# fhfonsecaa/SG-GAN-TF2

Hardware: AMD Instinct MI355X
Metric: train-step images/sec (G+D fwd/bwd) at 512x256 (higher is better)
Workload: dtype bf16; 1 GPU; BASELINE configs[2]: cycle-mode train step (north_star unit: G_A->B + G_B->A + D_A + D_B, LSGAN + cycle-L1 + gradient-sensitive losses; 12G+14D conv MACs), 9-block ResNet generators, 512x256, batch 8/GPU, bf16 storage / f32 accumulate; mode=cycle, global_batch=8, height=256, width=512, parallelism=dp1, mixed_gradient_chain=False

## Files before the change

sg-gan-tf2_amd/csrc/common.h:

```cpp
#pragma once
#include <hip/hip_runtime.h>
#include <hip/hip_ext.h>
#include <stdint.h>
#include <atomic>
#include <type_traits>
#include "../../include/sggan.h"

typedef __bf16 bf16;
typedef __attribute__((ext_vector_type(8))) __bf16 bf16x8;
typedef __attribute__((ext_vector_type(4))) __bf16 bf16x4;
typedef __attribute__((ext_vector_type(4))) float f32x4;
typedef __attribute__((ext_vector_type(4))) uint32_t u32x4;
typedef __attribute__((ext_vector_type(2))) uint32_t u32x2;

#define SGG_WAVE 64

template <typename T> struct ET;
template <> struct ET<float> {
    static constexpr int VEC = 4;
    __device__ static inline void unpack(const u32x4& c, float* f) {
#pragma unroll
        for (int i = 0; i < 4; ++i) f[i] = __uint_as_float(c[i]);
    }
    __device__ static inline u32x4 pack(const float* f) {
// ... 149 lines not shown
    const uint32_t m = __builtin_amdgcn_readfirstlane((uint32_t)(uintptr_t)lds_wave_base);
    const uint64_t b = (uint64_t)(uintptr_t)sbase;
    const uint64_t sb = (uint64_t)(uint32_t)__builtin_amdgcn_readfirstlane((uint32_t)b) |
                        ((uint64_t)(uint32_t)__builtin_amdgcn_readfirstlane((uint32_t)(b >> 32)) << 32);
    asm volatile("s_mov_b32 m0, %2\n\ts_nop 0\n\tglobal_load_lds_dwordx4 %0, %1" ::"v"(voff), "s"(sb), "s"(m) : "memory", "m0");
}

__device__ inline void dma4_to_lds(const void* gsrc, __attribute__((address_space(3))) void* lds_wave_base) {
    const uint32_t m = __builtin_amdgcn_readfirstlane((uint32_t)(uintptr_t)lds_wave_base);
    asm volatile("s_mov_b32 m0, %1\n\ts_nop 0\n\tglobal_load_lds_dword %0, off" ::"v"(gsrc), "s"(m) : "memory", "m0");
}
template <int N> __device__ inline void sgg_wait_vm() {
    static_assert(N >= 0 && N < 64, "vmcnt is a 6-bit counter");
    __builtin_amdgcn_s_waitcnt((N & 15) | ((N >> 4) << 14) | 0x0F70);
    asm volatile("" ::: "memory");
}
#define SGG_WAIT_VM0() sgg_wait_vm<0>()
#define SGG_WAIT_LGKM0() do { __builtin_amdgcn_s_waitcnt(0xC07F); asm volatile("" ::: "memory"); } while (0)

static inline int sgg_check_launch() { return hipGetLastError() == hipSuccess ? SGG_OK : SGG_ELAUNCH; }

static inline int sgg_lds_attr(const void* kern, int bytes, std::atomic<uint64_t>& done) {
    int dev = 0;
    if (hipGetDevice(&dev) != hipSuccess) return SGG_ELAUNCH;
    const uint64_t bit = 1ull << (dev & 63);
    if (done.load(std::memory_order_acquire) & bit) return SGG_OK;
    if (hipFuncSetAttribute(kern, hipFuncAttributeMaxDynamicSharedMemorySize, bytes) != hipSuccess) { (void)hipGetLastError(); return SGG_ELAUNCH; }
    done.fetch_or(bit, std::memory_order_release);
    return SGG_OK;
}
#define SGG_LDS_ATTR(kern, bytes)                                                        \
    do {                                                                                 \
        static std::atomic<uint64_t> sgg_attr_done_{0};                                  \
        int sgg_attr_rc_ = sgg_lds_attr((const void*)(kern), (int)(bytes), sgg_attr_done_); \
        if (sgg_attr_rc_) return sgg_attr_rc_;                                           \
    } while (0)

struct SggTimedLaunch { hipEvent_t start = nullptr, stop = nullptr; int consumed = 0; };
SggTimedLaunch& sgg_timed_launch();
template <typename F, typename... Args>
static inline void sgg_launch_timed(F kern, dim3 grid, dim3 block, unsigned lds, hipStream_t s, Args... args) {
    SggTimedLaunch& t = sgg_timed_launch();
    if (t.start && !t.consumed) {
        hipExtLaunchKernelGGL(kern, grid, block, lds, s, t.start, t.stop, 0, args...);
        t.consumed = 1;
    } else {
        hipLaunchKernelGGL(kern, grid, block, lds, s, args...);
    }
}

struct SggConfig {
    int halo3 = 1, s2halo = 1, w9 = 1, w9s2 = 1, stem_dgrad_halo = 1, wgrad_rowfast = 1, n7 = 1;
    int in_fused_maxhw = -1;
    int ablate = 0;
};
const SggConfig& sgg_config();
static inline size_t align_up(size_t v, size_t a) { return (v + a - 1) / a * a; }
```

sg-gan-tf2_amd/csrc/conv.hip:

```cpp
#include "conv_internal.h"

const SggConfig& sgg_config() {
#ifdef SGG_LAB
    static const SggConfig cfg = [] {
        SggConfig c;
        auto rd = [](const char* n, int dflt) { const char* e = getenv(n); return e ? atoi(e) : dflt; };
        c.halo3 = rd("SGG_HALO3", c.halo3);
        c.s2halo = rd("SGG_S2HALO", c.s2halo);
        c.w9 = rd("SGG_W9", c.w9);
        c.w9s2 = rd("SGG_W9S2", c.w9s2);
        c.stem_dgrad_halo = rd("SGG_STEM_DGRAD_HALO", c.stem_dgrad_halo);
        c.n7 = rd("SGG_N7", c.n7);
        c.wgrad_rowfast = rd("SGG_WGRAD_ROWFAST", c.wgrad_rowfast);
        c.in_fused_maxhw = rd("SGG_IN_FUSED_MAXHW", c.in_fused_maxhw);
        c.ablate = rd("SGG_ABLATE", 0);
        return c;
    }();
    return cfg;
#else
    static const SggConfig cfg;
    return cfg;
#endif
}

template <typename T>
__device__ inline u32x4 chunk_add(const u32x4& a, const u32x4& b) {
    float fa[ET<T>::VEC], fb[ET<T>::VEC];
    ET<T>::unpack(a, fa);
    ET<T>::unpack(b, fb);
#pragma unroll
    for (int i = 0; i < ET<T>::VEC; ++i) fa[i] += fb[i];
    return ET<T>::pack(fa);
}

__device__ inline int reflect_preimages(int h, int H, int p, int* j) {
    int n = 0;
    j[n++] = h + p;
    if (h >= 1 && h <= p) j[n++] = p - h;
    if (h >= H - 1 - p && h <= H - 2) j[n++] = p + 2 * (H - 1) - h;
    return n;
}

template <typename T, int BN, int WGM>
__global__ __launch_bounds__(256) void conv_border_fold_kernel(ConvArgs a) {
    constexpr int VEC = ET<T>::VEC;
    constexpr int ES = (int)sizeof(T);
    constexpr int BM = 64;
    constexpr int WGN = 4 / WGM;
    constexpr int WM = BM / WGM, WN = BN / WGN;
    constexpr int MI = WM / 16, NI = WN / 16;
    constexpr int PA = BM / 32;
    constexpr int QA = (BN + 31) / 32;
    static_assert(WM % 16 == 0 && WN % 16 == 0, "tile shape");

    extern __shared__ __attribute__((aligned(16))) char smem[];
    char* sP = smem;
    char* sQ = smem + BM * 128;

    const int tid = threadIdx.x, lane = tid & 63, wave = __builtin_amdgcn_readfirstlane(tid >> 6);
    const int wm = wave / WGN, wn = wave % WGN;
    const int SC = a.K, DC = a.C;
    const int cpv = SC / VEC;
    const int wrow = a.R * a.S * SC;
    const int p = a.pad_t, p2 = 2 * p;
    const int Bimg = p2 * a.W + (a.H - p2) * p2;
    const int M = a.N * Bimg;
    const int m0 = blockIdx.x * BM, n0 = blockIdx.y * BN;
// ... 2092 lines not shown
```

sg-gan-tf2_amd/csrc/norm.hip:

```cpp
#include "common.h"
#include <type_traits>

#define IN_U (BWD ? 2 : 4)
template <typename T> using InAcc = typename std::conditional<std::is_same<T, float>::value, double, float>::type;

struct InSplit { const float* gamma2; const float* beta2; float* dgamma2; float* dbeta2; int nsplit; };
static inline InSplit in_nosplit() { InSplit s; s.gamma2 = nullptr; s.beta2 = nullptr; s.dgamma2 = nullptr; s.dbeta2 = nullptr; s.nsplit = 0x7fffffff; return s; }

#ifndef IN_NT
#define IN_NT 15
#endif
template <typename T, typename TG, bool NT = false>
__device__ inline void in_load_grad(const char* dy, size_t elem, float* gv) {
    if constexpr (std::is_same<T, TG>::value) {
        ET<T>::unpack(NT ? ld16_nt(dy + elem * sizeof(T)) : ld16(dy + elem * sizeof(T)), gv);
    } else {
        static_assert(std::is_same<TG, float>::value && ET<T>::VEC == 8, "mixed mode: f32 gradient of a bf16 tensor");
        ET<float>::unpack(ld16(dy + elem * 4), gv);
        ET<float>::unpack(ld16(dy + elem * 4 + 16), gv + 4);
    }
}

static inline int in_rows_per_chunk(int64_t HW) {
    int64_t r = (HW + 127) / 128;
// ... 182 lines not shown
            auto sweep = [&](auto res_c) {
                constexpr bool RES = decltype(res_c)::value;
                auto one = [&](const u32x4& xr, const u32x4& rr, const float* gv, size_t off) {
                    float xv[VEC], o[VEC];
                    ET<T>::unpack(xr, xv);
                    if (!BWD) {
#pragma unroll
                        for (int e = 0; e < VEC; ++e) o[e] = act_apply_c<ACT>(xv[e] * A[e] + B[e], leak);
                        if (RES) {
                            float rv[VEC];
                            ET<T>::unpack(rr, rv);
#pragma unroll
                            for (int e = 0; e < VEC; ++e) o[e] += rv[e];
                        }
                    } else {
#pragma unroll
                        for (int e = 0; e < VEC; ++e) {
                            float xh = (xv[e] - mu[e]) * rs[e];
                            float g = gv[e] * act_grad_c<ACT>(gm[e] * xh + bt[e], leak);
                            o[e] = A[e] * (g - m1[e] - xh * m2[e]);
                        }
                    }
                    st16(out + off, ET<T>::pack(o));
                };
                const size_t base = ((size_t)n * HW * C + (size_t)cv * VEC) * sizeof(T), pstep = (size_t)C * sizeof(T);
                int64_t p = p0 + prow;
                for (; p + (IN_U - 1) * rows < p1; p += IN_U * rows) {
                    u32x4 xr[IN_U], rr[IN_U];
                    float gv[IN_U][BWD ? VEC : 1];
#pragma unroll
                    for (int u = 0; u < IN_U; ++u) {
                        const size_t off = base + (size_t)(p + u * rows) * pstep;
                        xr[u] = (IN_NT & (BWD ? 2 : 1)) ? ld16_nt(x + off) : ld16(x + off);
                        if (RES) rr[u] = (IN_NT & 8) ? ld16_nt(residual + off) : ld16(residual + off);
                    }
                    if (BWD) {
#pragma unroll
                        for (int u = 0; u < IN_U; ++u) in_load_grad<T, TG>(dy, (base + (size_t)(p + u * rows) * pstep) / sizeof(T), gv[u]);
                    }
#pragma unroll
                    for (int u = 0; u < IN_U; ++u) one(xr[u], rr[u], gv[u], base + (size_t)(p + u * rows) * pstep);
                }
                for (; p < p1; p += rows) {
                    const size_t off = base + (size_t)p * pstep;
                    float gv[BWD ? VEC : 1];
                    const u32x4 xr = (IN_NT & (BWD ? 2 : 1)) ? ld16_nt(x + off) : ld16(x + off);
                    u32x4 rr = xr;
                    if (RES) rr = (IN_NT & 8) ? ld16_nt(residual + off) : ld16(residual + off);
                    if (BWD) in_load_grad<T, TG, (IN_NT & 4) != 0>(dy, off / sizeof(T), gv);
                    one(xr, rr, gv, off);
                }
            };
            if (!BWD && residual) sweep(std::true_type{}); else sweep(std::false_type{});
        });
    }
}


#define IN_CVB 4
#define IN_FUSED_MAXHW 512

template <typename T, bool BWD>
__global__ __launch_bounds__(256) void in_fused_small_kernel(const char* x, const char* dy, const char* residual, const float* gamma,
                                                             const float* beta, float* stats, float* tot, char* out,
                                                             int64_t HW, int C, float eps, int act, float leak, InSplit sp) {
    constexpr int VEC = ET<T>::VEC;
    constexpr int ROWS = 256 / IN_CVB;
    const int CV = C / VEC;
    const int n = blockIdx.y;
    if (n >= sp.nsplit) { gamma = sp.gamma2; beta = sp.beta2; }
    const int cvl = threadIdx.x % IN_CVB, prow = threadIdx.x / IN_CVB;
    const int cv = blockIdx.x * IN_CVB + cvl;
    const bool live = cv < CV;
    using AccT = InAcc<T>;
    __shared__ AccT red[256][2 * VEC + 1];
    __shared__ float sh_a[IN_CVB * VEC], sh_b[IN_CVB * VEC];

    float mu[VEC], rs[VEC], gm[VEC], bt[VEC];
    if (live) {
#pragma unroll
        for (int e = 0; e < VEC; ++e) {
            const int c = cv * VEC + e;
            gm[e] = gamma[c]; bt[e] = beta[c];
            if (BWD) { mu[e] = stats[((size_t)n * C + c) * 2]; rs[e] = stats[((size_t)n * C + c) * 2 + 1]; }
        }
    }
    AccT s1[VEC], s2[VEC];
#pragma unroll
    for (int e = 0; e < VEC; ++e) s1[e] = s2[e] = (AccT)0;
    if (live)
        for (int64_t p = prow; p < HW; p += ROWS) {
            const size_t off = (((size_t)n * HW + p) * C + (size_t)cv * VEC) * sizeof(T);
            float xv[VEC];
            ET<T>::unpack(ld16(x + off), xv);
            if (!BWD) {
#pragma unroll
                for (int e = 0; e < VEC; ++e) { s1[e] += (AccT)xv[e]; s2[e] += (AccT)xv[e] * (AccT)xv[e]; }
            } else {
                float gv[VEC];
                ET<T>::unpack(ld16(dy + off), gv);
#pragma unroll
                for (int e = 0; e < VEC; ++e) {
                    const float xh = (xv[e] - mu[e]) * rs[e];
                    const float g = gv[e] * (act == SGG_ACT_RELU ? (gm[e] * xh + bt[e] > 0.f ? 1.f : 0.f) : act == SGG_ACT_LRELU ? (gm[e] * xh + bt[e] > 0.f ? 1.f : leak) : 1.f);
                    s1[e] += (AccT)g; s2[e] += (AccT)g * (AccT)xh;
                }
// ... 154 lines not shown
                    const u32x4 dzr = ET<T>::pack(dz);
                    st16(dz_out + off, dzr);
                    ET<T>::unpack(dzr, dz);
#pragma unroll
                    for (int e = 0; e < VEC; ++e) {
                        const float xh = (xv[e] - mu[e]) * rs[e];
                        s1[e] += (AccT)dz[e]; s2[e] += (AccT)dz[e] * (AccT)xh;
                    }
                };
                const size_t base = ((size_t)n * HW * C + (size_t)cv * VEC) * sizeof(T), pstep = (size_t)C * sizeof(T);
                int64_t p = p0 + prow;
                for (; p + rows < p1; p += 2 * rows) {
                    u32x4 xr[2], gr[2], yr[2];
#pragma unroll
                    for (int u = 0; u < 2; ++u) {
                        const size_t off = base + (size_t)(p + u * rows) * pstep;
                        xr[u] = ld16(x + off); gr[u] = ld16_nt(dy + off); yr[u] = ld16_nt(y + off);
                    }
#pragma unroll
                    for (int u = 0; u < 2; ++u) one(xr[u], gr[u], yr[u], base + (size_t)(p + u * rows) * pstep);
                }
                for (; p < p1; p += rows) {
                    const size_t off = base + (size_t)p * pstep;
                    one(ld16(x + off), ld16_nt(dy + off), ld16_nt(y + off), off);
                }
            });
        }
#pragma unroll
        for (int e = 0; e < VEC; ++e) { red[threadIdx.x][e] = s1[e]; red[threadIdx.x][VEC + e] = s2[e]; }
        __syncthreads();
        for (int item = threadIdx.x; item < lanes * VEC; item += 256) {
            const int l = item / VEC, e = item % VEC;
            AccT a = (AccT)0, b = (AccT)0;
            for (int r = 0; r < rows; ++r) { a += red[r * lanes + l][e]; b += red[r * lanes + l][VEC + e]; }
            const int c = (cvb + l) * VEC + e;
            const size_t o = (((size_t)n * chunks + chunk) * C + c) * 2;
            partial[o] = (float)a; partial[o + 1] = (float)b;
        }
        __syncthreads();
    }
}

static bool in_use_fused(int64_t HW) {
    const int mx = sgg_config().in_fused_maxhw;
    return HW <= (mx >= 0 ? mx : IN_FUSED_MAXHW);
}

static int in_rows_per_block(int N, int64_t HW, int C, int vec) {
    int64_t r = HW * N / 2048;
    if (r < 64) r = 64;
    if (r > 4096) r = 4096;
    return (int)r;
}

extern "C" {

size_t sgg_instnorm_workspace(int N, int64_t HW, int C) {
    if (N <= 0 || HW <= 0 || C <= 0) return 0;
    return ((size_t)N * in_chunks(HW) * C * 2 + (size_t)N * C * 4) * sizeof(float);
}

static int instnorm_fwd_impl(const void* x, const float* gamma, const float* beta, const void* residual, void* y, float* stats,
                     int N, int64_t HW, int C, float eps, int act, float leak, int dtype, void* ws, size_t ws_bytes, void* stream, InSplit sp) {
    if (!x || !gamma || !beta || !y || !stats || N <= 0 || HW <= 0 || C <= 0 || C % SGG_CPAD) return SGG_EINVAL;
    if (act == SGG_ACT_TANH) return SGG_EUNSUPPORTED;
    if (!ws || ws_bytes < sgg_instnorm_workspace(N, HW, C)) return SGG_EWORKSPACE;
    hipStream_t s = (hipStream_t)stream;
    if (dtype != SGG_BF16 && dtype != SGG_F32) return SGG_EINVAL;
    if (in_use_fused(HW)) {
        const int vec = dtype == SGG_BF16 ? 8 : 4;
        dim3 gf((unsigned)((C / vec + IN_CVB - 1) / IN_CVB), N);
        if (dtype == SGG_BF16) hipLaunchKernelGGL((in_fused_small_kernel<bf16, false>), gf, dim3(256), 0, s, (const char*)x, nullptr, (const char*)residual, gamma, beta, stats, nullptr, (char*)y, HW, C, eps, act, leak, sp);
        else hipLaunchKernelGGL((in_fused_small_kernel<float, false>), gf, dim3(256), 0, s, (const char*)x, nullptr, (const char*)residual, gamma, beta, stats, nullptr, (char*)y, HW, C, eps, act, leak, sp);
        return sgg_check_launch();
    }
    int chunks = in_chunks(HW);
    float* partial = (float*)ws;
    int rpb = in_rows_per_block(N, HW, C, 0);
    dim3 gp(chunks, N), ga((unsigned)((HW + rpb - 1) / rpb), N);
    if (dtype == SGG_BF16) {
        hipLaunchKernelGGL((in_partial_kernel<bf16, false>), gp, dim3(256), 0, s, (const char*)x, nullptr, gamma, beta, nullptr, partial, HW, C, chunks, in_rows_per_chunk(HW), act, leak, sp);
        hipLaunchKernelGGL(in_finalize_fwd_kernel, dim3((C + FIN_CH - 1) / FIN_CH, N), dim3(1024), 0, s, partial, stats, HW, C, chunks, eps);
        sgg_launch_timed(in_apply_kernel<bf16, false>, ga, dim3(256), 0u, s, (const char*)x, (const char*)nullptr, (const char*)residual, gamma, beta, (const float*)stats, (const float*)nullptr, (char*)y, HW, C, rpb, act, leak, InParamGrad{}, sp);
    } else if (dtype == SGG_F32) {
        hipLaunchKernelGGL((in_partial_kernel<float, false>), gp, dim3(256), 0, s, (const char*)x, nullptr, gamma, beta, nullptr, partial, HW, C, chunks, in_rows_per_chunk(HW), act, leak, sp);
        hipLaunchKernelGGL(in_finalize_fwd_kernel, dim3((C + FIN_CH - 1) / FIN_CH, N), dim3(1024), 0, s, partial, stats, HW, C, chunks, eps);
        hipLaunchKernelGGL((in_apply_kernel<float, false>), ga, dim3(256), 0, s, (const char*)x, nullptr, (const char*)residual, gamma, beta, stats, nullptr, (char*)y, HW, C, rpb, act, leak, InParamGrad{}, sp);
    } else return SGG_EINVAL;
    return sgg_check_launch();
}

static int instnorm_fwd_partial_impl(const void* x, const float* gamma, const float* beta, const void* residual, void* y, float* stats,
                             const float* partial, int chunks, int N, int64_t HW, int C, float eps, int act, float leak, int dtype,
                             void* stream, InSplit sp) {
    if (!x || !gamma || !beta || !y || !stats || !partial || chunks <= 0 || N <= 0 || HW <= 0 || C <= 0 || C % SGG_CPAD) return SGG_EINVAL;
    if (act == SGG_ACT_TANH) return SGG_EUNSUPPORTED;
    if (dtype != SGG_BF16 && dtype != SGG_F32) return SGG_EINVAL;
    hipStream_t s = (hipStream_t)stream;
    int rpb = in_rows_per_block(N, HW, C, 0);
    dim3 ga((unsigned)((HW + rpb - 1) / rpb), N);
    hipLaunchKernelGGL(in_finalize_fwd_kernel, dim3((C + FIN_CH - 1) / FIN_CH, N), dim3(1024), 0, s, partial, stats, HW, C, chunks, eps);
    if (dtype == SGG_BF16) sgg_launch_timed(in_apply_kernel<bf16, false>, ga, dim3(256), 0u, s, (const char*)x, (const char*)nullptr, (const char*)residual, gamma, beta, (const float*)stats, (const float*)nullptr, (char*)y, HW, C, rpb, act, leak, InParamGrad{}, sp);
    else hipLaunchKernelGGL((in_apply_kernel<float, false>), ga, dim3(256), 0, s, (const char*)x, nullptr, (const char*)residual, gamma, beta, stats, nullptr, (char*)y, HW, C, rpb, act, leak, InParamGrad{}, sp);
    return sgg_check_launch();
}

static int instnorm_bwd_impl(const void* dy, const void* x, const float* gamma, const float* beta, const float* stats, void* dx,
                     float* dgamma, float* dbeta, int N, int64_t HW, int C, int C_real, int accumulate, int act, float leak,
                     int dtype, void* ws, size_t ws_bytes, void* stream, InSplit sp) {
    if (!dy || !x || !gamma || !beta || !stats || !dx || !dgamma || !dbeta || N <= 0 || HW <= 0 || C <= 0 || C % SGG_CPAD || C_real <= 0 || C_real > C) return SGG_EINVAL;
    if (act == SGG_ACT_TANH) return SGG_EUNSUPPORTED;
    if (!ws || ws_bytes < sgg_instnorm_workspace(N, HW, C)) return SGG_EWORKSPACE;
    hipStream_t s = (hipStream_t)stream;
    int chunks = in_chunks(HW);
    float* partial = (float*)ws;
    float* sums = partial + (size_t)N * chunks * C * 2;
    float* tot = sums + (size_t)N * C * 2;
    int rpb = in_rows_per_block(N, HW, C, 0);
    dim3 gp(chunks, N), ga((unsigned)((HW + rpb - 1) / rpb), N);
    const InParamGrad pg{tot, dgamma, dbeta, N, C_real, accumulate};
    if (dtype != SGG_BF16 && dtype != SGG_F32) return SGG_EINVAL;
    if (in_use_fused(HW)) {
        const int vec = dtype == SGG_BF16 ? 8 : 4;
        dim3 gf((unsigned)((C / vec + IN_CVB - 1) / IN_CVB), N);
        if (dtype == SGG_BF16) hipLaunchKernelGGL((in_fused_small_kernel<bf16, true>), gf, dim3(256), 0, s, (const char*)x, (const char*)dy, nullptr, gamma, beta, (float*)stats, tot, (char*)dx, HW, C, 0.f, act, leak, sp);
        else hipLaunchKernelGGL((in_fused_small_kernel<float, true>), gf, dim3(256), 0, s, (const char*)x, (const char*)dy, nullptr, gamma, beta, (float*)stats, tot, (char*)dx, HW, C, 0.f, act, leak, sp);
        hipLaunchKernelGGL(in_param_grad_kernel, dim3(1), dim3(256), 0, s, pg, C, sp);
        return sgg_check_launch();
    }
    if (dtype == SGG_BF16) {
        hipLaunchKernelGGL((in_partial_kernel<bf16, true>), gp, dim3(256), 0, s, (const char*)x, (const char*)dy, gamma, beta, stats, partial, HW, C, chunks, in_rows_per_chunk(HW), act, leak, sp);
        hipLaunchKernelGGL(in_finalize_bwd_kernel, dim3((C + FIN_CH - 1) / FIN_CH, N), dim3(1024), 0, s, partial, sums, tot, HW, C, chunks);
        hipLaunchKernelGGL((in_apply_kernel<bf16, true>), ga, dim3(256), 0, s, (const char*)x, (const char*)dy, nullptr, gamma, beta, stats, sums, (char*)dx, HW, C, rpb, act, leak, pg, sp);
    } else if (dtype == SGG_F32) {
        hipLaunchKernelGGL((in_partial_kernel<float, true>), gp, dim3(256), 0, s, (const char*)x, (const char*)dy, gamma, beta, stats, partial, HW, C, chunks, in_rows_per_chunk(HW), act, leak, sp);
        hipLaunchKernelGGL(in_finalize_bwd_kernel, dim3((C + FIN_CH - 1) / FIN_CH, N), dim3(1024), 0, s, partial, sums, tot, HW, C, chunks);
        hipLaunchKernelGGL((in_apply_kernel<float, true>), ga, dim3(256), 0, s, (const char*)x, (const char*)dy, nullptr, gamma, beta, stats, sums, (char*)dx, HW, C, rpb, act, leak, pg, sp);
    } else return SGG_EINVAL;
    return sgg_check_launch();
}

static int instnorm_bwd_mixed_impl(const float* dy, const void* x, const float* gamma, const float* beta, const float* stats, void* dx,
                           float* dgamma, float* dbeta, int N, int64_t HW, int C, int C_real, int accumulate, int act, float leak,
                           void* ws, size_t ws_bytes, void* stream, InSplit sp) {
    if (!dy || !x || !gamma || !beta || !stats || !dx || !dgamma || !dbeta || N <= 0 || HW <= 0 || C <= 0 || C % SGG_CPAD || C_real <= 0 || C_real > C) return SGG_EINVAL;
    if (act == SGG_ACT_TANH) return SGG_EUNSUPPORTED;
    if (!ws || ws_bytes < sgg_instnorm_workspace(N, HW, C)) return SGG_EWORKSPACE;
    hipStream_t s = (hipStream_t)stream;
    int chunks = in_chunks(HW);
    float* partial = (float*)ws;
    float* sums = partial + (size_t)N * chunks * C * 2;
    float* tot = sums + (size_t)N * C * 2;
    int rpb = in_rows_per_block(N, HW, C, 0);
    dim3 gp(chunks, N), ga((unsigned)((HW + rpb - 1) / rpb), N);
    const InParamGrad pg{tot, dgamma, dbeta, N, C_real, accumulate};
    hipLaunchKernelGGL((in_partial_kernel<bf16, true, float>), gp, dim3(256), 0, s, (const char*)x, (const char*)dy, gamma, beta, stats, partial, HW, C, chunks, in_rows_per_chunk(HW), act, leak, sp);
    hipLaunchKernelGGL(in_finalize_bwd_kernel, dim3((C + FIN_CH - 1) / FIN_CH, N), dim3(1024), 0, s, partial, sums, tot, HW, C, chunks);
    hipLaunchKernelGGL((in_apply_kernel<bf16, true, float>), ga, dim3(256), 0, s, (const char*)x, (const char*)dy, nullptr, gamma, beta, stats, sums, (char*)dx, HW, C, rpb, act, leak, pg, sp);
    return sgg_check_launch();
}

static int instnorm_bwd_partial_impl(const void* dy, const void* x, const float* gamma, const float* beta, const float* stats, void* dx,
                             float* dgamma, float* dbeta, const float* partial, int chunks, int N, int64_t HW, int C, int C_real,
                             int accumulate, int act, float leak, int dtype, void* ws, size_t ws_bytes, void* stream, InSplit sp) {
    if (!dy || !x || !gamma || !beta || !stats || !dx || !dgamma || !dbeta || !partial || chunks <= 0 || N <= 0 || HW <= 0 || C <= 0 ||
        C % SGG_CPAD || C_real <= 0 || C_real > C) return SGG_EINVAL;
    if (act == SGG_ACT_TANH) return SGG_EUNSUPPORTED;
    if (dtype != SGG_BF16 && dtype != SGG_F32) return SGG_EINVAL;
    if (!ws || ws_bytes < (size_t)N * C * 4 * sizeof(float)) return SGG_EWORKSPACE;
    hipStream_t s = (hipStream_t)stream;
    float* sums = (float*)ws;
    float* tot = sums + (size_t)N * C * 2;
    int rpb = in_rows_per_block(N, HW, C, 0);
    dim3 ga((unsigned)((HW + rpb - 1) / rpb), N);
    const InParamGrad pg{tot, dgamma, dbeta, N, C_real, accumulate};
    hipLaunchKernelGGL(in_finalize_bwd_kernel, dim3((C + FIN_CH - 1) / FIN_CH, N), dim3(1024), 0, s, partial, sums, tot, HW, C, chunks);
    if (dtype == SGG_BF16) hipLaunchKernelGGL((in_apply_kernel<bf16, true>), ga, dim3(256), 0, s, (const char*)x, (const char*)dy, nullptr, gamma, beta, stats, sums, (char*)dx, HW, C, rpb, act, leak, pg, sp);
    else hipLaunchKernelGGL((in_apply_kernel<float, true>), ga, dim3(256), 0, s, (const char*)x, (const char*)dy, nullptr, gamma, beta, stats, sums, (char*)dx, HW, C, rpb, act, leak, pg, sp);
    return sgg_check_launch();
}

int sgg_instnorm_fwd(const void* x, const float* gamma, const float* beta, const void* residual, void* y, float* stats,
                     int N, int64_t HW, int C, float eps, int act, float leak, int dtype, void* ws, size_t ws_bytes, void* stream) {
    return instnorm_fwd_impl(x, gamma, beta, residual, y, stats, N, HW, C, eps, act, leak, dtype, ws, ws_bytes, stream, in_nosplit());
}
int sgg_instnorm_fwd_partial(const void* x, const float* gamma, const float* beta, const void* residual, void* y, float* stats,
                             const float* partial, int chunks, int N, int64_t HW, int C, float eps, int act, float leak, int dtype,
                             void* stream) {
    return instnorm_fwd_partial_impl(x, gamma, beta, residual, y, stats, partial, chunks, N, HW, C, eps, act, leak, dtype, stream, in_nosplit());
}
int sgg_instnorm_bwd(const void* dy, const void* x, const float* gamma, const float* beta, const float* stats, void* dx,
                     float* dgamma, float* dbeta, int N, int64_t HW, int C, int C_real, int accumulate, int act, float leak,
                     int dtype, void* ws, size_t ws_bytes, void* stream) {
    return instnorm_bwd_impl(dy, x, gamma, beta, stats, dx, dgamma, dbeta, N, HW, C, C_real, accumulate, act, leak, dtype, ws, ws_bytes, stream, in_nosplit());
}
int sgg_instnorm_bwd_mixed(const float* dy, const void* x, const float* gamma, const float* beta, const float* stats, void* dx,
                           float* dgamma, float* dbeta, int N, int64_t HW, int C, int C_real, int accumulate, int act, float leak,
                           void* ws, size_t ws_bytes, void* stream) {
    return instnorm_bwd_mixed_impl(dy, x, gamma, beta, stats, dx, dgamma, dbeta, N, HW, C, C_real, accumulate, act, leak, ws, ws_bytes, stream, in_nosplit());
}
int sgg_instnorm_bwd_partial(const void* dy, const void* x, const float* gamma, const float* beta, const float* stats, void* dx,
                             float* dgamma, float* dbeta, const float* partial, int chunks, int N, int64_t HW, int C, int C_real,
                             int accumulate, int act, float leak, int dtype, void* ws, size_t ws_bytes, void* stream) {
    return instnorm_bwd_partial_impl(dy, x, gamma, beta, stats, dx, dgamma, dbeta, partial, chunks, N, HW, C, C_real, accumulate, act, leak, dtype, ws, ws_bytes, stream, in_nosplit());
}
int sgg_instnorm_finalize(const float* partial, int chunks, float* stats, int N, int64_t HW, int C, float eps, void* stream) {
    if (!partial || !stats || chunks <= 0 || N <= 0 || HW <= 0 || C <= 0 || C % SGG_CPAD) return SGG_EINVAL;
    hipLaunchKernelGGL(in_finalize_fwd_kernel, dim3((C + FIN_CH - 1) / FIN_CH, N), dim3(1024), 0, (hipStream_t)stream, partial, stats, HW, C, chunks, eps);
    return sgg_check_launch();
}
static inline int in_pair_ok(const float* g2, const float* b2, int nsplit, int N) { return g2 && b2 && nsplit > 0 && nsplit < N; }
int sgg_instnorm_fwd_pair(const void* x, const float* gamma, const float* beta, const float* gamma2, const float* beta2, int nsplit,
                          const void* residual, void* y, float* stats, int N, int64_t HW, int C, float eps, int act, float leak,
                          int dtype, void* ws, size_t ws_bytes, void* stream) {
    if (!in_pair_ok(gamma2, beta2, nsplit, N)) return SGG_EINVAL;
    InSplit sp = in_nosplit(); sp.gamma2 = gamma2; sp.beta2 = beta2; sp.nsplit = nsplit;
    return instnorm_fwd_impl(x, gamma, beta, residual, y, stats, N, HW, C, eps, act, leak, dtype, ws, ws_bytes, stream, sp);
}
int sgg_instnorm_fwd_partial_pair(const void* x, const float* gamma, const float* beta, const float* gamma2, const float* beta2, int nsplit,
                                  const void* residual, void* y, float* stats, const float* partial, int chunks, int N, int64_t HW, int C,
                                  float eps, int act, float leak, int dtype, void* stream) {
    if (!in_pair_ok(gamma2, beta2, nsplit, N)) return SGG_EINVAL;
    InSplit sp = in_nosplit(); sp.gamma2 = gamma2; sp.beta2 = beta2; sp.nsplit = nsplit;
    return instnorm_fwd_partial_impl(x, gamma, beta, residual, y, stats, partial, chunks, N, HW, C, eps, act, leak, dtype, stream, sp);
}
int sgg_instnorm_bwd_pair(const void* dy, const void* x, const float* gamma, const float* beta, const float* gamma2, const float* beta2,
                          int nsplit, const float* stats, void* dx, float* dgamma, float* dbeta, float* dgamma2, float* dbeta2,
                          int N, int64_t HW, int C, int C_real, int accumulate, int act, float leak, int dtype,
                          void* ws, size_t ws_bytes, void* stream) {
    if (!in_pair_ok(gamma2, beta2, nsplit, N) || !dgamma2 || !dbeta2) return SGG_EINVAL;
    InSplit sp; sp.gamma2 = gamma2; sp.beta2 = beta2; sp.dgamma2 = dgamma2; sp.dbeta2 = dbeta2; sp.nsplit = nsplit;
    return instnorm_bwd_impl(dy, x, gamma, beta, stats, dx, dgamma, dbeta, N, HW, C, C_real, accumulate, act, leak, dtype, ws, ws_bytes, stream, sp);
}

static int instnorm_fwd_skip_apply(const void* x, const float* gamma, const float* beta, const void* skip, void* y, const float* stats,
                                   int N, int64_t HW, int C, int act, float leak, int dtype, hipStream_t s, InSplit sp) {
    const int rpb = in_rows_per_block(N, HW, C, 0);
    const dim3 ga((unsigned)((HW + rpb - 1) / rpb), N);
    if (dtype == SGG_BF16) hipLaunchKernelGGL(in_apply_skip_kernel<bf16>, ga, dim3(256), 0, s, (const char*)x, (const char*)skip, gamma, beta, stats, (char*)y, HW, C, rpb, act, leak, sp);
    else hipLaunchKernelGGL(in_apply_skip_kernel<float>, ga, dim3(256), 0, s, (const char*)x, (const char*)skip, gamma, beta, stats, (char*)y, HW, C, rpb, act, leak, sp);
    return sgg_check_launch();
}
static int instnorm_fwd_skip_impl(const void* x, const float* gamma, const float* beta, const void* skip, void* y, float* stats,
                                  int N, int64_t HW, int C, float eps, int act, float leak, int dtype, void* ws, size_t ws_bytes, void* stream,
                                  InSplit sp) {
    if (!x || !gamma || !beta || !skip || !y || !stats || N <= 0 || HW <= 0 || C <= 0 || C % SGG_CPAD) return SGG_EINVAL;
    if (act == SGG_ACT_TANH) return SGG_EUNSUPPORTED;
    if (dtype != SGG_BF16 && dtype != SGG_F32) return SGG_EINVAL;
    if (!ws || ws_bytes < sgg_instnorm_workspace(N, HW, C)) return SGG_EWORKSPACE;
    hipStream_t s = (hipStream_t)stream;
    const int chunks = in_chunks(HW);
    float* partial = (float*)ws;
    const dim3 gp(chunks, N);
    if (dtype == SGG_BF16) hipLaunchKernelGGL((in_partial_kernel<bf16, false>), gp, dim3(256), 0, s, (const char*)x, nullptr, gamma, beta, nullptr, partial, HW, C, chunks, in_rows_per_chunk(HW), act, leak, sp);
    else hipLaunchKernelGGL((in_partial_kernel<float, false>), gp, dim3(256), 0, s, (const char*)x, nullptr, gamma, beta, nullptr, partial, HW, C, chunks, in_rows_per_chunk(HW), act, leak, sp);
    hipLaunchKernelGGL(in_finalize_fwd_kernel, dim3((C + FIN_CH - 1) / FIN_CH, N), dim3(1024), 0, s, partial, stats, HW, C, chunks, eps);
    return instnorm_fwd_skip_apply(x, gamma, beta, skip, y, stats, N, HW, C, act, leak, dtype, s, sp);
}
static int instnorm_fwd_skip_partial_impl(const void* x, const float* gamma, const float* beta, const void* skip, void* y, float* stats,
                                          const float* partial, int chunks, int N, int64_t HW, int C, float eps, int act, float leak, int dtype,
                                          void* stream, InSplit sp) {
    if (!x || !gamma || !beta || !skip || !y || !stats || !partial || chunks <= 0 || N <= 0 || HW <= 0 || C <= 0 || C % SGG_CPAD) return SGG_EINVAL;
    if (act == SGG_ACT_TANH) return SGG_EUNSUPPORTED;
    if (dtype != SGG_BF16 && dtype != SGG_F32) return SGG_EINVAL;
    hipStream_t s = (hipStream_t)stream;
    hipLaunchKernelGGL(in_finalize_fwd_kernel, dim3((C + FIN_CH - 1) / FIN_CH, N), dim3(1024), 0, s, partial, stats, HW, C, chunks, eps);
    return instnorm_fwd_skip_apply(x, gamma, beta, skip, y, stats, N, HW, C, act, leak, dtype, s, sp);
}
static int instnorm_bwd_skip_impl(const void* dy, const void* y, const void* x, const float* gamma, const float* beta, const float* stats,
                                  void* dx, void* dskip, float* dgamma, float* dbeta, int N, int64_t HW, int C, int C_real, int accumulate,
                                  int act, float leak, int dtype, void* ws, size_t ws_bytes, void* stream, InSplit sp) {
    if (!dy || !y || !x || !gamma || !beta || !stats || !dx || !dskip || !dgamma || !dbeta || N <= 0 || HW <= 0 || C <= 0 ||
        C % SGG_CPAD || C_real <= 0 || C_real > C) return SGG_EINVAL;
    if (act == SGG_ACT_TANH) return SGG_EUNSUPPORTED;
    if (dtype != SGG_BF16 && dtype != SGG_F32) return SGG_EINVAL;
    if (dx == dskip || dx == dy || dx == x) return SGG_EINVAL;
    if (!ws || ws_bytes < sgg_instnorm_workspace(N, HW, C)) return SGG_EWORKSPACE;
    hipStream_t s = (hipStream_t)stream;
    const int chunks = in_chunks(HW);
    float* partial = (float*)ws;
    float* sums = partial + (size_t)N * chunks * C * 2;
    float* tot = sums + (size_t)N * C * 2;
    const int rpb = in_rows_per_block(N, HW, C, 0);
    const dim3 gp(chunks, N), ga((unsigned)((HW + rpb - 1) / rpb), N);
    const InParamGrad pg{tot, dgamma, dbeta, N, C_real, accumulate};
    if (dtype == SGG_BF16) {
        hipLaunchKernelGGL(in_skip_bwd_partial_kernel<bf16>, gp, dim3(256), 0, s, (const char*)x, (const char*)dy, (const char*)y, stats, (char*)dskip, partial, HW, C, chunks, in_rows_per_chunk(HW), act, leak);
        hipLaunchKernelGGL(in_finalize_bwd_kernel, dim3((C + FIN_CH - 1) / FIN_CH, N), dim3(1024), 0, s, partial, sums, tot, HW, C, chunks);
        hipLaunchKernelGGL((in_apply_kernel<bf16, true>), ga, dim3(256), 0, s, (const char*)x, (const char*)dskip, nullptr, gamma, beta, stats, sums, (char*)dx, HW, C, rpb, (int)SGG_ACT_NONE, 0.f, pg, sp);
    } else {
        hipLaunchKernelGGL(in_skip_bwd_partial_kernel<float>, gp, dim3(256), 0, s, (const char*)x, (const char*)dy, (const char*)y, stats, (char*)dskip, partial, HW, C, chunks, in_rows_per_chunk(HW), act, leak);
        hipLaunchKernelGGL(in_finalize_bwd_kernel, dim3((C + FIN_CH - 1) / FIN_CH, N), dim3(1024), 0, s, partial, sums, tot, HW, C, chunks);
        hipLaunchKernelGGL((in_apply_kernel<float, true>), ga, dim3(256), 0, s, (const char*)x, (const char*)dskip, nullptr, gamma, beta, stats, sums, (char*)dx, HW, C, rpb, (int)SGG_ACT_NONE, 0.f, pg, sp);
    }
    return sgg_check_launch();
}
int sgg_instnorm_fwd_skip(const void* x, const float* gamma, const float* beta, const void* skip, void* y, float* stats,
                          int N, int64_t HW, int C, float eps, int act, float leak, int dtype, void* ws, size_t ws_bytes, void* stream) {
    return instnorm_fwd_skip_impl(x, gamma, beta, skip, y, stats, N, HW, C, eps, act, leak, dtype, ws, ws_bytes, stream, in_nosplit());
}
int sgg_instnorm_fwd_skip_partial(const void* x, const float* gamma, const float* beta, const void* skip, void* y, float* stats,
                                  const float* partial, int chunks, int N, int64_t HW, int C, float eps, int act, float leak, int dtype,
                                  void* stream) {
    return instnorm_fwd_skip_partial_impl(x, gamma, beta, skip, y, stats, partial, chunks, N, HW, C, eps, act, leak, dtype, stream, in_nosplit());
}
int sgg_instnorm_bwd_skip(const void* dy, const void* y, const void* x, const float* gamma, const float* beta, const float* stats,
                          void* dx, void* dskip, float* dgamma, float* dbeta, int N, int64_t HW, int C, int C_real, int accumulate,
                          int act, float leak, int dtype, void* ws, size_t ws_bytes, void* stream) {
    return instnorm_bwd_skip_impl(dy, y, x, gamma, beta, stats, dx, dskip, dgamma, dbeta, N, HW, C, C_real, accumulate, act, leak, dtype,
                                  ws, ws_bytes, stream, in_nosplit());
}
int sgg_instnorm_fwd_skip_pair(const void* x, const float* gamma, const float* beta, const float* gamma2, const float* beta2, int nsplit,
                               const void* skip, void* y, float* stats, int N, int64_t HW, int C, float eps, int act, float leak,
                               int dtype, void* ws, size_t ws_bytes, void* stream) {
    if (!in_pair_ok(gamma2, beta2, nsplit, N)) return SGG_EINVAL;
    InSplit sp = in_nosplit(); sp.gamma2 = gamma2; sp.beta2 = beta2; sp.nsplit = nsplit;
    return instnorm_fwd_skip_impl(x, gamma, beta, skip, y, stats, N, HW, C, eps, act, leak, dtype, ws, ws_bytes, stream, sp);
}
int sgg_instnorm_fwd_skip_partial_pair(const void* x, const float* gamma, const float* beta, const float* gamma2, const float* beta2, int nsplit,
                                       const void* skip, void* y, float* stats, const float* partial, int chunks, int N, int64_t HW, int C,
                                       float eps, int act, float leak, int dtype, void* stream) {
    if (!in_pair_ok(gamma2, beta2, nsplit, N)) return SGG_EINVAL;
    InSplit sp = in_nosplit(); sp.gamma2 = gamma2; sp.beta2 = beta2; sp.nsplit = nsplit;
    return instnorm_fwd_skip_partial_impl(x, gamma, beta, skip, y, stats, partial, chunks, N, HW, C, eps, act, leak, dtype, stream, sp);
}
int sgg_instnorm_bwd_skip_pair(const void* dy, const void* y, const void* x, const float* gamma, const float* beta, const float* gamma2,
                               const float* beta2, int nsplit, const float* stats, void* dx, void* dskip, float* dgamma, float* dbeta,
                               float* dgamma2, float* dbeta2, int N, int64_t HW, int C, int C_real, int accumulate, int act, float leak,
                               int dtype, void* ws, size_t ws_bytes, void* stream) {
    if (!in_pair_ok(gamma2, beta2, nsplit, N) || !dgamma2 || !dbeta2) return SGG_EINVAL;
    InSplit sp; sp.gamma2 = gamma2; sp.beta2 = beta2; sp.dgamma2 = dgamma2; sp.dbeta2 = dbeta2; sp.nsplit = nsplit;
    return instnorm_bwd_skip_impl(dy, y, x, gamma, beta, stats, dx, dskip, dgamma, dbeta, N, HW, C, C_real, accumulate, act, leak, dtype,
                                  ws, ws_bytes, stream, sp);
}

}
```

Before: 288.4 images/sec.

## Add LDS-ring prefetch kernel for bf16 instance-norm backward apply

Adds a new bf16 backward apply kernel for instance norm. It streams x and dy into a per-wave LDS ring of depth 4 using global_load_lds DMA, with explicit vmcnt waits to keep several loads in flight. Launches are routed through new helpers, and the ring kernel uses its own grid sizing, targeting about 1024 blocks. The aim is to hide memory latency in this bandwidth-bound pass, at the cost of extra LDS use, hand-written waitcnt logic and a changed block geometry.

Measured after the change: 289.2 images/sec, median of 6. No clear change (+0.3%).

```diff
diff --git a/sg-gan-tf2_amd/csrc/common.h b/sg-gan-tf2_amd/csrc/common.h
--- a/sg-gan-tf2_amd/csrc/common.h
+++ b/sg-gan-tf2_amd/csrc/common.h
@@ -225,6 +225,7 @@
 struct SggConfig {
     int halo3 = 1, s2halo = 1, w9 = 1, w9s2 = 1, stem_dgrad_halo = 1, wgrad_rowfast = 1, n7 = 1;
     int in_fused_maxhw = -1;
+    int in_bwd_ring = 1;
     int ablate = 0;
 };
 const SggConfig& sgg_config();
diff --git a/sg-gan-tf2_amd/csrc/conv.hip b/sg-gan-tf2_amd/csrc/conv.hip
--- a/sg-gan-tf2_amd/csrc/conv.hip
+++ b/sg-gan-tf2_amd/csrc/conv.hip
@@ -13,6 +13,7 @@
         c.n7 = rd("SGG_N7", c.n7);
         c.wgrad_rowfast = rd("SGG_WGRAD_ROWFAST", c.wgrad_rowfast);
         c.in_fused_maxhw = rd("SGG_IN_FUSED_MAXHW", c.in_fused_maxhw);
+        c.in_bwd_ring = rd("SGG_IN_BWD_RING", c.in_bwd_ring);
         c.ablate = rd("SGG_ABLATE", 0);
         return c;
     }();
diff --git a/sg-gan-tf2_amd/csrc/norm.hip b/sg-gan-tf2_amd/csrc/norm.hip
--- a/sg-gan-tf2_amd/csrc/norm.hip
+++ b/sg-gan-tf2_amd/csrc/norm.hip
@@ -258,6 +258,99 @@
                 }
             };
             if (!BWD && residual) sweep(std::true_type{}); else sweep(std::false_type{});
+        });
+    }
+}
+
+#ifndef IN_RING_D
+#define IN_RING_D 4
+#endif
+#ifndef IN_APPLY_BLOCKS
+#define IN_APPLY_BLOCKS 1024
+#endif
+
+template <bool NT> __device__ inline void in_dma16(const void* gsrc, u32x4* slot) {
+    typedef __attribute__((address_space(3))) void* lds_ptr;
+    if constexpr (NT) {
+        const uint32_t m = __builtin_amdgcn_readfirstlane((uint32_t)(uintptr_t)(lds_ptr)slot);
+        asm volatile("s_mov_b32 m0, %1\n\ts_nop 0\n\tglobal_load_lds_dwordx4 %0, off nt" ::"v"(gsrc), "s"(m) : "memory", "m0");
+    } else {
+        dma16_to_lds(gsrc, (lds_ptr)slot);
+    }
+}
+__device__ inline void in_wait_vm_dyn(int n) {
+    switch (n) {
+#define IN_W(k) case k: sgg_wait_vm<k>(); break;
+        IN_W(0) IN_W(1) IN_W(2) IN_W(3) IN_W(4) IN_W(5) IN_W(6) IN_W(7) IN_W(8) IN_W(9) IN_W(10) IN_W(11) IN_W(12) IN_W(13) IN_W(14) IN_W(15)
+#undef IN_W
+        default: sgg_wait_vm<16>(); break;
+    }
+}
+
+__global__ __launch_bounds__(256) void in_apply_bwd_ring_kernel(const char* x, const char* dy, const float* gamma, const float* beta,
+                                                                const float* stats, const float* sums, char* out, int64_t HW, int C,
+                                                                int rows_per_block, int act, float leak, InParamGrad pg, InSplit sp) {
+    using T = bf16;
+    constexpr int VEC = ET<T>::VEC, D = IN_RING_D, LD = 2;
+    const int CV = C / VEC;
+    const int n = blockIdx.y;
+    if (blockIdx.x == 0 && blockIdx.y == 0) in_param_grad(pg, C, sp);
+    if (n >= sp.nsplit) { gamma = sp.gamma2; beta = sp.beta2; }
+    const int64_t p0 = (int64_t)blockIdx.x * rows_per_block;
+    const int64_t p1 = p0 + rows_per_block < HW ? p0 + rows_per_block : HW;
+    __shared__ u32x4 ring[4][D][LD][64];
+    const int wave = threadIdx.x >> 6, lane = threadIdx.x & 63;
+    for (int cvb = 0; cvb < CV; cvb += 256) {
+        const int lanes = CV - cvb < 256 ? CV - cvb : 256;
+        const int rows = 256 / lanes;
+        const int cv = cvb + (int)(threadIdx.x % lanes), prow = threadIdx.x / lanes;
+        if (prow >= rows) continue;
+        const int trips = (int)((p1 - p0 + rows - 1) / rows);
+        act_dispatch(act, [&](auto act_c) {
+            constexpr int ACT = decltype(act_c)::value;
+            const size_t base = ((size_t)n * HW * C + (size_t)cv * VEC) * sizeof(T), pstep = (size_t)C * sizeof(T);
+            auto issue = [&](int k) {
+                int64_t p = p0 + prow + (int64_t)k * rows;
+                if (p >= p1) p = p1 - 1;
+                const size_t off = base + (size_t)p * pstep;
+                u32x4* s = &ring[wave][k % D][0][0];
+                in_dma16<(IN_NT & 2) != 0>(x + off, s);
+                in_dma16<false>(dy + off, s + 64);
+            };
+            const int fill = trips < D ? trips : D;
+            for (int k = 0; k < fill; ++k) issue(k);
+            float A[VEC], mu[VEC], rs[VEC], gm[VEC], bt[VEC], m1[VEC], m2[VEC];
+#pragma unroll
+            for (int e = 0; e < VEC; ++e) {
+                int c = cv * VEC + e;
+                mu[e] = stats[((size_t)n * C + c) * 2]; rs[e] = stats[((size_t)n * C + c) * 2 + 1];
+                gm[e] = gamma[c]; bt[e] = beta[c];
+                A[e] = gm[e] * rs[e];
+                m1[e] = sums[((size_t)n * C + c) * 2]; m2[e] = sums[((size_t)n * C + c) * 2 + 1];
+            }
+            SGG_WAIT_VM0();
+            for (int i = 0; i < trips; ++i) {
+                const int rem = trips - 1 - i;
+                if (i >= D && rem >= D - 1) sgg_wait_vm<LD * (D - 1) + D>();
+                else in_wait_vm_dyn(LD * (rem < D - 1 ? rem : D - 1) + (i < D ? i : D));
+                const u32x4* s = &ring[wave][i % D][0][lane];
+                const u32x4 xr = s[0], gr = s[64];
+                SGG_WAIT_LGKM0();
+                if (i + D < trips) issue(i + D);
+                const int64_t p = p0 + prow + (int64_t)i * rows;
+                if (p < p1) {
+                    float xv[VEC], gv[VEC], o[VEC];
+                    ET<T>::unpack(xr, xv);
+                    ET<T>::unpack(gr, gv);
+#pragma unroll
+                    for (int e = 0; e < VEC; ++e) {
+                        float xh = (xv[e] - mu[e]) * rs[e];
+                        float g = gv[e] * act_grad_c<ACT>(gm[e] * xh + bt[e], leak);
+                        o[e] = A[e] * (g - m1[e] - xh * m2[e]);
+                    }
+                    st16(out + base + (size_t)p * pstep, ET<T>::pack(o));
+                }
+            }
         });
     }
 }
@@ -518,8 +611,50 @@
     if (r > 4096) r = 4096;
     return (int)r;
 }
+static int in_ring_rows_per_block(int N, int64_t HW) {
+    int64_t r = (HW * N + IN_APPLY_BLOCKS - 1) / IN_APPLY_BLOCKS;
+    if (r < 64) r = 64;
+    if (r > HW) r = HW;
+    return (int)r;
+}
+
+template <typename T, bool BWD, typename TG = T>
+static void in_launch_partial(hipStream_t s, const void* x, const void* dy, const float* gamma, const float* beta, const float* stats,
+                              float* partial, int N, int64_t HW, int C, int chunks, int act, float leak, InSplit sp) {
+    hipLaunchKernelGGL((in_partial_kernel<T, BWD, TG>), dim3(chunks, N), dim3(256), 0, s, (const char*)x, (const char*)dy, gamma, beta,
+                       stats, partial, HW, C, chunks, in_rows_per_chunk(HW), act, leak, sp);
+}
+template <typename T, bool BWD, typename TG = T>
+static void in_launch_apply(hipStream_t s, const void* x, const void* dy, const void* residual, const float* gamma, const float* beta,
+                            const float* stats, const float* sums, void* out, int N, int64_t HW, int C, int act, float leak,
+                            InParamGrad pg, InSplit sp) {
+    if constexpr (BWD && std::is_same<T, bf16>::value && std::is_same<TG, bf16>::value) {
+        if (sgg_config().in_bwd_ring) {
+            const int rpb = in_ring_rows_per_block(N, HW);
+            hipLaunchKernelGGL(in_apply_bwd_ring_kernel, dim3((unsigned)((HW + rpb - 1) / rpb), N), dim3(256), 0, s, (const char*)x, (const char*)dy,
+                               gamma, beta, stats, sums, (char*)out, HW, C, rpb, act, leak, pg, sp);
+            return;
+        }
+    }
+    {
+        const int rpb = in_rows_per_block(N, HW, C, 0);
+        const dim3 ga((unsigned)((HW + rpb - 1) / rpb), N);
+        if constexpr (!BWD && std::is_same<T, bf16>::value)
+            sgg_launch_timed(in_apply_kernel<T, BWD, TG>, ga, dim3(256), 0u, s, (const char*)x, (const char*)dy, (const char*)residual, gamma, beta, stats, sums, (char*)out, HW, C, rpb, act, leak, pg, sp);
+        else
+            hipLaunchKernelGGL((in_apply_kernel<T, BWD, TG>), ga, dim3(256), 0, s, (const char*)x, (const char*)dy, (const char*)residual, gamma, beta, stats, sums, (char*)out, HW, C, rpb, act, leak, pg, sp);
+    }
+}
 
 extern "C" {
+
+int sgg_instnorm_bwd_apply_geometry(int N, int64_t HW, int C, int dtype, int mixed, int* depth, int* pixels_per_block) {
+    if (N <= 0 || HW <= 0 || C <= 0 || (dtype != SGG_BF16 && dtype != SGG_F32) || !depth || !pixels_per_block) return SGG_EINVAL;
+    const bool ring = dtype == SGG_BF16 && !mixed && sgg_config().in_bwd_ring;
+    *depth = ring ? IN_RING_D : 0;
+    *pixels_per_block = ring ? in_ring_rows_per_block(N, HW) : in_rows_per_block(N, HW, C, 0);
+    return SGG_OK;
+}
 
 size_t sgg_instnorm_workspace(int N, int64_t HW, int C) {
     if (N <= 0 || HW <= 0 || C <= 0) return 0;
@@ -542,16 +677,14 @@
     }
     int chunks = in_chunks(HW);
     float* partial = (float*)ws;
-    int rpb = in_rows_per_block(N, HW, C, 0);
-    dim3 gp(chunks, N), ga((unsigned)((HW + rpb - 1) / rpb), N);
     if (dtype == SGG_BF16) {
-        hipLaunchKernelGGL((in_partial_kernel<bf16, false>), gp, dim3(256), 0, s, (const char*)x, nullptr, gamma, beta, nullptr, partial, HW, C, chunks, in_rows_per_chunk(HW), act, leak, sp);
+        in_launch_partial<bf16, false>(s, x, nullptr, gamma, beta, nullptr, partial, N, HW, C, chunks, act, leak, sp);
         hipLaunchKernelGGL(in_finalize_fwd_kernel, dim3((C + FIN_CH - 1) / FIN_CH, N), dim3(1024), 0, s, partial, stats, HW, C, chunks, eps);
-        sgg_launch_timed(in_apply_kernel<bf16, false>, ga, dim3(256), 0u, s, (const char*)x, (const char*)nullptr, (const char*)residual, gamma, beta, (const float*)stats, (const float*)nullptr, (char*)y, HW, C, rpb, act, leak, InParamGrad{}, sp);
+        in_launch_apply<bf16, false>(s, x, nullptr, residual, gamma, beta, stats, nullptr, y, N, HW, C, act, leak, InParamGrad{}, sp);
     } else if (dtype == SGG_F32) {
-        hipLaunchKernelGGL((in_partial_kernel<float, false>), gp, dim3(256), 0, s, (const char*)x, nullptr, gamma, beta, nullptr, partial, HW, C, chunks, in_rows_per_chunk(HW), act, leak, sp);
+        in_launch_partial<float, false>(s, x, nullptr, gamma, beta, nullptr, partial, N, HW, C, chunks, act, leak, sp);
         hipLaunchKernelGGL(in_finalize_fwd_kernel, dim3((C + FIN_CH - 1) / FIN_CH, N), dim3(1024), 0, s, partial, stats, HW, C, chunks, eps);
-        hipLaunchKernelGGL((in_apply_kernel<float, false>), ga, dim3(256), 0, s, (const char*)x, nullptr, (const char*)residual, gamma, beta, stats, nullptr, (char*)y, HW, C, rpb, act, leak, InParamGrad{}, sp);
+        in_launch_apply<float, false>(s, x, nullptr, residual, gamma, beta, stats, nullptr, y, N, HW, C, act, leak, InParamGrad{}, sp);
     } else return SGG_EINVAL;
     return sgg_check_launch();
 }
@@ -563,11 +696,9 @@
     if (act == SGG_ACT_TANH) return SGG_EUNSUPPORTED;
     if (dtype != SGG_BF16 && dtype != SGG_F32) return SGG_EINVAL;
     hipStream_t s = (hipStream_t)stream;
-    int rpb = in_rows_per_block(N, HW, C, 0);
-    dim3 ga((unsigned)((HW + rpb - 1) / rpb), N);
     hipLaunchKernelGGL(in_finalize_fwd_kernel, dim3((C + FIN_CH - 1) / FIN_CH, N), dim3(1024), 0, s, partial, stats, HW, C, chunks, eps);
-    if (dtype == SGG_BF16) sgg_launch_timed(in_apply_kernel<bf16, false>, ga, dim3(256), 0u, s, (const char*)x, (const char*)nullptr, (const char*)residual, gamma, beta, (const float*)stats, (const float*)nullptr, (char*)y, HW, C, rpb, act, leak, InParamGrad{}, sp);
-    else hipLaunchKernelGGL((in_apply_kernel<float, false>), ga, dim3(256), 0, s, (const char*)x, nullptr, (const char*)residual, gamma, beta, stats, nullptr, (char*)y, HW, C, rpb, act, leak, InParamGrad{}, sp);
+    if (dtype == SGG_BF16) in_launch_apply<bf16, false>(s, x, nullptr, residual, gamma, beta, stats, nullptr, y, N, HW, C, act, leak, InParamGrad{}, sp);
+    else in_launch_apply<float, false>(s, x, nullptr, residual, gamma, beta, stats, nullptr, y, N, HW, C, act, leak, InParamGrad{}, sp);
     return sgg_check_launch();
 }
 
@@ -582,8 +713,6 @@
     float* partial = (float*)ws;
     float* sums = partial + (size_t)N * chunks * C * 2;
     float* tot = sums + (size_t)N * C * 2;
-    int rpb = in_rows_per_block(N, HW, C, 0);
-    dim3 gp(chunks, N), ga((unsigned)((HW + rpb - 1) / rpb), N);
     const InParamGrad pg{tot, dgamma, dbeta, N, C_real, accumulate};
     if (dtype != SGG_BF16 && dtype != SGG_F32) return SGG_EINVAL;
     if (in_use_fused(HW)) {
@@ -595,13 +724,13 @@
         return sgg_check_launch();
     }
     if (dtype == SGG_BF16) {
-        hipLaunchKernelGGL((in_partial_kernel<bf16, true>), gp, dim3(256), 0, s, (const char*)x, (const char*)dy, gamma, beta, stats, partial, HW, C, chunks, in_rows_per_chunk(HW), act, leak, sp);
+        in_launch_partial<bf16, true>(s, x, dy, gamma, beta, stats, partial, N, HW, C, chunks, act, leak, sp);
         hipLaunchKernelGGL(in_finalize_bwd_kernel, dim3((C + FIN_CH - 1) / FIN_CH, N), dim3(1024), 0, s, partial, sums, tot, HW, C, chunks);
-        hipLaunchKernelGGL((in_apply_kernel<bf16, true>), ga, dim3(256), 0, s, (const char*)x, (const char*)dy, nullptr, gamma, beta, stats, sums, (char*)dx, HW, C, rpb, act, leak, pg, sp);
+        in_launch_apply<bf16, true>(s, x, dy, nullptr, gamma, beta, stats, sums, dx, N, HW, C, act, leak, pg, sp);
     } else if (dtype == SGG_F32) {
-        hipLaunchKernelGGL((in_partial_kernel<float, true>), gp, dim3(256), 0, s, (const char*)x, (const char*)dy, gamma, beta, stats, partial, HW, C, chunks, in_rows_per_chunk(HW), act, leak, sp);
+        in_launch_partial<float, true>(s, x, dy, gamma, beta, stats, partial, N, HW, C, chunks, act, leak, sp);
         hipLaunchKernelGGL(in_finalize_bwd_kernel, dim3((C + FIN_CH - 1) / FIN_CH, N), dim3(1024), 0, s, partial, sums, tot, HW, C, chunks);
-        hipLaunchKernelGGL((in_apply_kernel<float, true>), ga, dim3(256), 0, s, (const char*)x, (const char*)dy, nullptr, gamma, beta, stats, sums, (char*)dx, HW, C, rpb, act, leak, pg, sp);
+        in_launch_apply<float, true>(s, x, dy, nullptr, gamma, beta, stats, sums, dx, N, HW, C, act, leak, pg, sp);
     } else return SGG_EINVAL;
     return sgg_check_launch();
 }
@@ -617,12 +746,10 @@
     float* partial = (float*)ws;
     float* sums = partial + (size_t)N * chunks * C * 2;
     float* tot = sums + (size_t)N * C * 2;
-    int rpb = in_rows_per_block(N, HW, C, 0);
-    dim3 gp(chunks, N), ga((unsigned)((HW + rpb - 1) / rpb), N);
     const InParamGrad pg{tot, dgamma, dbeta, N, C_real, accumulate};
-    hipLaunchKernelGGL((in_partial_kernel<bf16, true, float>), gp, dim3(256), 0, s, (const char*)x, (const char*)dy, gamma, beta, stats, partial, HW, C, chunks, in_rows_per_chunk(HW), act, leak, sp);
+    in_launch_partial<bf16, true, float>(s, x, dy, gamma, beta, stats, partial, N, HW, C, chunks, act, leak, sp);
     hipLaunchKernelGGL(in_finalize_bwd_kernel, dim3((C + FIN_CH - 1) / FIN_CH, N), dim3(1024), 0, s, partial, sums, tot, HW, C, chunks);
-    hipLaunchKernelGGL((in_apply_kernel<bf16, true, float>), ga, dim3(256), 0, s, (const char*)x, (const char*)dy, nullptr, gamma, beta, stats, sums, (char*)dx, HW, C, rpb, act, leak, pg, sp);
+    in_launch_apply<bf16, true, float>(s, x, dy, nullptr, gamma, beta, stats, sums, dx, N, HW, C, act, leak, pg, sp);
     return sgg_check_launch();
 }
 
@@ -637,12 +764,10 @@
     hipStream_t s = (hipStream_t)stream;
     float* sums = (float*)ws;
     float* tot = sums + (size_t)N * C * 2;
-    int rpb = in_rows_per_block(N, HW, C, 0);
-    dim3 ga((unsigned)((HW + rpb - 1) / rpb), N);
     const InParamGrad pg{tot, dgamma, dbeta, N, C_real, accumulate};
     hipLaunchKernelGGL(in_finalize_bwd_kernel, dim3((C + FIN_CH - 1) / FIN_CH, N), dim3(1024), 0, s, partial, sums, tot, HW, C, chunks);
-    if (dtype == SGG_BF16) hipLaunchKernelGGL((in_apply_kernel<bf16, true>), ga, dim3(256), 0, s, (const char*)x, (const char*)dy, nullptr, gamma, beta, stats, sums, (char*)dx, HW, C, rpb, act, leak, pg, sp);
-    else hipLaunchKernelGGL((in_apply_kernel<float, true>), ga, dim3(256), 0, s, (const char*)x, (const char*)dy, nullptr, gamma, beta, stats, sums, (char*)dx, HW, C, rpb, act, leak, pg, sp);
+    if (dtype == SGG_BF16) in_launch_apply<bf16, true>(s, x, dy, nullptr, gamma, beta, stats, sums, dx, N, HW, C, act, leak, pg, sp);
+    else in_launch_apply<float, true>(s, x, dy, nullptr, gamma, beta, stats, sums, dx, N, HW, C, act, leak, pg, sp);
     return sgg_check_launch();
 }
 
@@ -717,9 +842,8 @@
     hipStream_t s = (hipStream_t)stream;
     const int chunks = in_chunks(HW);
     float* partial = (float*)ws;
-    const dim3 gp(chunks, N);
-    if (dtype == SGG_BF16) hipLaunchKernelGGL((in_partial_kernel<bf16, false>), gp, dim3(256), 0, s, (const char*)x, nullptr, gamma, beta, nullptr, partial, HW, C, chunks, in_rows_per_chunk(HW), act, leak, sp);
-    else hipLaunchKernelGGL((in_partial_kernel<float, false>), gp, dim3(256), 0, s, (const char*)x, nullptr, gamma, beta, nullptr, partial, HW, C, chunks, in_rows_per_chunk(HW), act, leak, sp);
+    if (dtype == SGG_BF16) in_launch_partial<bf16, false>(s, x, nullptr, gamma, beta, nullptr, partial, N, HW, C, chunks, act, leak, sp);
+    else in_launch_partial<float, false>(s, x, nullptr, gamma, beta, nullptr, partial, N, HW, C, chunks, act, leak, sp);
     hipLaunchKernelGGL(in_finalize_fwd_kernel, dim3((C + FIN_CH - 1) / FIN_CH, N), dim3(1024), 0, s, partial, stats, HW, C, chunks, eps);
     return instnorm_fwd_skip_apply(x, gamma, beta, skip, y, stats, N, HW, C, act, leak, dtype, s, sp);
 }
@@ -747,17 +871,16 @@
     float* partial = (float*)ws;
     float* sums = partial + (size_t)N * chunks * C * 2;
     float* tot = sums + (size_t)N * C * 2;
-    const int rpb = in_rows_per_block(N, HW, C, 0);
-    const dim3 gp(chunks, N), ga((unsigned)((HW + rpb - 1) / rpb), N);
+    const dim3 gp(chunks, N);
     const InParamGrad pg{tot, dgamma, dbeta, N, C_real, accumulate};
     if (dtype == SGG_BF16) {
         hipLaunchKernelGGL(in_skip_bwd_partial_kernel<bf16>, gp, dim3(256), 0, s, (const char*)x, (const char*)dy, (const char*)y, stats, (char*)dskip, partial, HW, C, chunks, in_rows_per_chunk(HW), act, leak);
         hipLaunchKernelGGL(in_finalize_bwd_kernel, dim3((C + FIN_CH - 1) / FIN_CH, N), dim3(1024), 0, s, partial, sums, tot, HW, C, chunks);
-        hipLaunchKernelGGL((in_apply_kernel<bf16, true>), ga, dim3(256), 0, s, (const char*)x, (const char*)dskip, nullptr, gamma, beta, stats, sums, (char*)dx, HW, C, rpb, (int)SGG_ACT_NONE, 0.f, pg, sp);
+        in_launch_apply<bf16, true>(s, x, dskip, nullptr, gamma, beta, stats, sums, dx, N, HW, C, (int)SGG_ACT_NONE, 0.f, pg, sp);
     } else {
         hipLaunchKernelGGL(in_skip_bwd_partial_kernel<float>, gp, dim3(256), 0, s, (const char*)x, (const char*)dy, (const char*)y, stats, (char*)dskip, partial, HW, C, chunks, in_rows_per_chunk(HW), act, leak);
         hipLaunchKernelGGL(in_finalize_bwd_kernel, dim3((C + FIN_CH - 1) / FIN_CH, N), dim3(1024), 0, s, partial, sums, tot, HW, C, chunks);
-        hipLaunchKernelGGL((in_apply_kernel<float, true>), ga, dim3(256), 0, s, (const char*)x, (const char*)dskip, nullptr, gamma, beta, stats, sums, (char*)dx, HW, C, rpb, (int)SGG_ACT_NONE, 0.f, pg, sp);
+        in_launch_apply<float, true>(s, x, dskip, nullptr, gamma, beta, stats, sums, dx, N, HW, C, (int)SGG_ACT_NONE, 0.f, pg, sp);
     }
     return sgg_check_launch();
 }
```
